# MIT-SPARK/Khronos

Measured on AMD Instinct MI355X. Metric: active-window frames/sec (+ Mvoxel-updates/sec) at 1280x720 RGB-D+labels, 2 cm voxels, higher is better.
Workload: dtype f32

## Files before the change

khronos_amd/csrc/khr_kernels_aux.h:

```cpp
#pragma once
#include <cstring>

#include "khr_device.h"

namespace khr {

#include "mc_table.inc"
__device__ int8_t g_mc_tri[256][16];
__device__ uint8_t g_mc_ntri[256];

constexpr uint64_t kSeedBit = kSeedFlag;

__global__ __launch_bounds__(256) void k_motion_pixels(DevMap m, DevParams p, DevFrame f, float md_max_range,
                                                      float min_z_world, uint64_t* __restrict__ keys, int ignore_epoch,
                                                      uint32_t* __restrict__ begin_band_count) {
  if (begin_band_count && blockIdx.x == 0) beginIntegrate(m, p.nvox, begin_band_count);
  const int i = blockIdx.x * blockDim.x + threadIdx.x;
  const bool in = i < f.W * f.H;
  uint64_t key = ~0ull;
  if (in)
    key = motionPixelKey(m, p, f.range[i], f.depth[i], i % f.W, i / f.W, f.fx, f.fy, f.cx, f.cy, f.Rw, f.tw, md_max_range,
                         min_z_world, ignore_epoch);
  if (in) keys[i] = key;
  const bool seed = (key != ~0ull) && (key & kSeedBit);
// ... 1548 lines not shown
  const uint32_t i = blockIdx.x * blockDim.x + threadIdx.x;
  if (i <= m.ht_mask) m.ht_keys[i] = kEmptyKey;
  if (i < m.capacity) {
    m.blk_flags[i] = 0u;
    m.mesh_desc[i] = MeshDesc{0u, 0u};
    m.free_slots[i] = i;
  }
  if (i < C_COUNT) m.counters[i] = i == C_N_FREE ? m.capacity : 0u;
  if (i < S_COUNT) m.stats[i] = 0ull;
}

__global__ __launch_bounds__(256) void k_block_flag_op(DevMap m, uint32_t and_mask, uint32_t or_mask) {
  const uint32_t s = blockIdx.x * blockDim.x + threadIdx.x;
  if (s >= m.counters[C_MAX_SLOT]) return;
  const uint32_t fl = m.blk_flags[s];
  if (fl & BLK_LIVE) m.blk_flags[s] = (fl & and_mask) | or_mask;
}

struct PackOut {
  float* dist;
  float* weight;
  uint32_t* color;
  uint64_t* last_obs;
  uint8_t* vflags;
  uint32_t* sem_label;
  uint64_t* last_occ;
  float* lik;
  int K, KS;
  uint64_t track_stamp;
};
template <int VPS>
__global__ __launch_bounds__(256) void k_pack_blocks(DevMap m, const uint32_t* __restrict__ slots, int n, PackOut o) {
  constexpr int NV = VPS * VPS * VPS;
  for (int b = blockIdx.x; b < n; b += gridDim.x) {
    const size_t src = static_cast<size_t>(slots[b]) * NV, dst = static_cast<size_t>(b) * NV;
    auto copy16 = [&](const void* s, void* d, size_t bytes) {
      const uint4* s4 = reinterpret_cast<const uint4*>(s);
      uint4* d4 = reinterpret_cast<uint4*>(d);
      for (size_t i = threadIdx.x; i < bytes / 16; i += 256) d4[i] = s4[i];
    };
    if (o.dist) copy16(m.dist + src, o.dist + dst, NV * 4);
    if (o.weight) copy16(m.weight + src, o.weight + dst, NV * 4);
    if (o.color) copy16(m.color + src, o.color + dst, NV * 4);
    if (o.last_obs) {
      const size_t sl = src / NV;
      for (int i = threadIdx.x; i < NV; i += 256) o.last_obs[dst + i] = lastObserved(m, sl, static_cast<uint32_t>(i), NV);
    }
    if (o.vflags) {
      const uint4* s4 = reinterpret_cast<const uint4*>(m.vflags + src);
      uint4* d4 = reinterpret_cast<uint4*>(o.vflags + dst);
      const uint32_t pm = VOX_PUBLIC_MASK * 0x01010101u;
      for (size_t i = threadIdx.x; i < NV / 16; i += 256) {
        const uint4 v = s4[i];
        d4[i] = make_uint4(v.x & pm, v.y & pm, v.z & pm, v.w & pm);
      }
    }
    if (o.sem_label) copy16(m.sem_label + src, o.sem_label + dst, NV * 4);
  }
}

__global__ __launch_bounds__(256) void k_snapshot_select(DevMap m, uint32_t* __restrict__ count, uint32_t* __restrict__ slots,
                                                        int4* __restrict__ index, uint32_t cap) {
  const uint32_t s = blockIdx.x * blockDim.x + threadIdx.x;
  bool take = false;
  if (s < m.counters[C_MAX_SLOT]) {
    const uint32_t fl = m.blk_flags[s];
    take = (fl & BLK_LIVE) && (fl & BLK_UPDATED);
  }
  const uint32_t pos = waveAggInc(count, take);
  if (take && pos < cap) {
    slots[pos] = s;
    index[pos] = m.blk_index[s];
  }
}
__global__ __launch_bounds__(256) void k_snapshot_index3(const int4* __restrict__ index, int32_t* __restrict__ out3, uint32_t n) {
  const uint32_t i = blockIdx.x * blockDim.x + threadIdx.x;
  if (i < n) {
    const int4 v = index[i];
    out3[3 * i] = v.x;
    out3[3 * i + 1] = v.y;
    out3[3 * i + 2] = v.z;
  }
}
template <int VPS>
__global__ __launch_bounds__(256) void k_snapshot_pack(DevMap m, const uint32_t* __restrict__ count, const uint32_t* __restrict__ slots,
                                                      uint32_t cap, PackOut o, volatile uint32_t* host_count, uint32_t ticket) {
  constexpr int NV = VPS * VPS * VPS;
  const uint32_t total = *count;
  const uint32_t n = min(total, cap);
  if (blockIdx.x == 0 && threadIdx.x == 0) {
    host_count[0] = total;
    __threadfence_system();
    host_count[1] = ticket;
    __threadfence_system();
  }
  for (uint32_t b = blockIdx.x; b < n; b += gridDim.x) {
    const size_t src = static_cast<size_t>(slots[b]) * NV, dst = static_cast<size_t>(b) * NV;
    auto copy16 = [&](const void* s, void* d, size_t bytes) {
      const uint4* s4 = reinterpret_cast<const uint4*>(s);
      uint4* d4 = reinterpret_cast<uint4*>(d);
      for (size_t i = threadIdx.x; i < bytes / 16; i += 256) d4[i] = s4[i];
    };
    if (o.dist) copy16(m.dist + src, o.dist + dst, NV * 4);
    if (o.weight) copy16(m.weight + src, o.weight + dst, NV * 4);
    if (o.color) copy16(m.color + src, o.color + dst, NV * 4);
    if (o.last_obs) {
      const size_t sl = src / NV;
      for (int i = threadIdx.x; i < NV; i += 256) o.last_obs[dst + i] = lastObserved(m, sl, static_cast<uint32_t>(i), NV);
    }
    if (o.vflags) {
      const uint4* s4 = reinterpret_cast<const uint4*>(m.vflags + src);
      uint4* d4 = reinterpret_cast<uint4*>(o.vflags + dst);
      const uint32_t pm = VOX_PUBLIC_MASK * 0x01010101u;
      for (size_t i = threadIdx.x; i < NV / 16; i += 256) {
        const uint4 v = s4[i];
        d4[i] = make_uint4(v.x & pm, v.y & pm, v.z & pm, v.w & pm);
      }
    }
    if (o.sem_label) copy16(m.sem_label + src, o.sem_label + dst, NV * 4);
    if (o.last_occ) {
      for (int i = threadIdx.x; i < NV; i += 256)
        o.last_occ[dst + i] = (m.vflags[src + i] & VOX_OCC) ? o.track_stamp : m.last_occ[src + i];
    }
    if (o.lik) {
      if (o.KS == o.K) copy16(m.lik + src * o.K, o.lik + dst * o.K, static_cast<size_t>(NV) * o.K * 4);
      else
        for (uint32_t i = threadIdx.x; i < static_cast<uint32_t>(NV) * static_cast<uint32_t>(o.K); i += 256) {
          const uint32_t v = i / static_cast<uint32_t>(o.K), k = i - v * static_cast<uint32_t>(o.K);
          o.lik[dst * o.K + i] = m.lik[(src + v) * o.KS + k];
        }
    }
  }
}

template <int VPS>
__global__ __launch_bounds__(256) void k_object_prune(DevMap m, DevParams p, float min_conf, float min_obs) {
  constexpr int NV = VPS * VPS * VPS;
  const uint32_t n_slots = m.counters[C_MAX_SLOT];
  uint32_t pruned = 0;
  for (uint32_t s = blockIdx.x; s < n_slots; s += gridDim.x) {
    if (!(m.blk_flags[s] & BLK_LIVE)) continue;
    const size_t o = static_cast<size_t>(s) * NV;
    bool touched = false;
    for (int lin = threadIdx.x; lin < NV; lin += 256) {
      const float d = m.dist[o + lin];
      if (d > 0.f) continue;
      float conf = 0.f;
      if (m.vflags[o + lin] & VOX_SEM_VALID) {
        const float l0 = m.lik[(static_cast<size_t>(s) * NV + lin) * p.KS + 0];
        const float l1 = m.lik[(static_cast<size_t>(s) * NV + lin) * p.KS + 1];
        const float total = l0 + l1;
        conf = total < min_obs ? -1.f : l1 / total;
      }
      if (conf < min_conf) {
        m.dist[o + lin] = p.trunc;
        ++pruned;
        touched = true;
      }
    }
    if (__any(touched) && (threadIdx.x & 63) == 0) atomicOr(&m.blk_flags[s], BLK_TRACK_DIRTY);
  }
#pragma unroll
  for (int o = 32; o > 0; o >>= 1) pruned += __shfl_down(pruned, o);
  if ((threadIdx.x & 63) == 0 && pruned) atomicAdd(&m.stats[S_PRUNED], static_cast<unsigned long long>(pruned));
}

constexpr int kDigestWords = 12;
__host__ __device__ inline uint64_t digestMix(uint64_t x) {
  x += 0x9e3779b97f4a7c15ull;
  x = (x ^ (x >> 30)) * 0xbf58476d1ce4e5b9ull;
  x = (x ^ (x >> 27)) * 0x94d049bb133111ebull;
  return x ^ (x >> 31);
}
__host__ __device__ inline uint64_t digestTerm(uint64_t key, uint32_t layer, uint64_t i, uint64_t value) {
  return digestMix(digestMix(key * 0x9e3779b97f4a7c15ull + static_cast<uint64_t>(layer) * 0x632be59bd9b4e019ull + i) ^ value);
}
__global__ __launch_bounds__(256) void k_map_digest(DevMap m, DevParams p, uint64_t track_stamp, unsigned long long* __restrict__ out) {
  const uint32_t n_slots = m.counters[C_MAX_SLOT];
  unsigned long long acc[kDigestWords];
#pragma unroll
  for (int l = 0; l < kDigestWords; ++l) acc[l] = 0ull;
  for (uint32_t s = blockIdx.x; s < n_slots; s += gridDim.x) {
    const uint32_t bf = m.blk_flags[s];
    if (!(bf & BLK_LIVE)) continue;
    const int4 bi = m.blk_index[s];
    const uint64_t key = packKey(bi.x, bi.y, bi.z);
    const size_t o = static_cast<size_t>(s) * p.nvox;
    for (int i = threadIdx.x; i < p.nvox; i += 256) {
      const uint8_t raw = m.vflags[o + i];
      acc[0] += digestTerm(key, 0, i, __float_as_uint(m.dist[o + i]));
      acc[1] += digestTerm(key, 1, i, __float_as_uint(m.weight[o + i]));
      acc[2] += digestTerm(key, 2, i, m.color[o + i]);
      const uint64_t lobs = p.with_tracking ? lastObserved(m, s, static_cast<uint32_t>(i), p.nvox) : 0ull;
      const uint64_t locc = p.with_tracking ? ((raw & VOX_OCC) ? track_stamp : m.last_occ[o + i]) : 0ull;
      acc[3] += digestTerm(key, 3, i, lobs);
      acc[4] += digestTerm(key, 4, i, locc);
      acc[5] += digestTerm(key, 5, i, raw & VOX_PUBLIC_MASK);
      acc[6] += digestTerm(key, 6, i, p.with_semantics ? m.sem_label[o + i] : 0u);
      if (p.with_semantics) {
        const bool valid = raw & VOX_SEM_VALID;
        const float* row = m.lik + (o + i) * p.KS;
        for (int k = 0; k < p.K; ++k)
          acc[7] += digestTerm(key, 7, static_cast<uint64_t>(k) * p.nvox + i, valid ? __float_as_uint(row[k]) : 0u);
      }
    }
    if (threadIdx.x == 0) {
      acc[8] += digestTerm(key, 8, 0, bf & 0xfu);
      acc[9] += digestMix(key);
      acc[10] += 1ull;
    }
  }
#pragma unroll
  for (int l = 0; l < kDigestWords; ++l) {
// ... 8 lines not shown
```

khronos_amd/csrc/khronos_amd.hip:

```cpp
#include <hip/hip_runtime.h>
#include <hip/hip_ext.h>
#include <hipcub/hipcub.hpp>

#include <algorithm>
#include <array>
#include <atomic>
#include <chrono>
#include <memory>
#include <mutex>
#include <cmath>
#include <cstdarg>
#include <cstdio>
#include <climits>
#include <cstring>
#include <cstdlib>
#include <functional>
#include <map>
#include <string>
#include <thread>
#include <tuple>
#include <unordered_map>
#include <vector>

#include "../../include/khronos_amd.h"
// ... 76 lines not shown
struct TimingRec {
  int which;
  Event a, b;
};

constexpr int kNumTimers = 13;
constexpr uint32_t kObjHead = 512;
constexpr uint32_t kCvHead = 8192;
constexpr int kGvReleaseGrid = 64;
constexpr uint32_t kCompCap = 1024, kCompHead = 64;

}

struct khr_ctx {
  khr_config cfg{};
  DevParams p{};
  DevMap m{};
  int device = 0;
  Stream stream;
  Stream aux_stream;
  Stream copy_stream;
  Stream snap_stream;
  Stream mc_stream;
  Stream h2d_stream;
  Event ev_aux, ev_aux_done;
  uint64_t aux_seq_issued = 0, aux_seq_done = 0, obj_seq = 0, cv_seq[3] = {0, 0, 0};
  std::vector<DevBuf<uint8_t>> allocs;
  std::vector<FrameSlot> slots;
  int next_slot = 0;
  std::unique_ptr<std::atomic<int>[]> slot_leases;
  uint32_t* d_work = nullptr;
  uint32_t* d_new = nullptr;
  uint32_t* d_ef = nullptr;
  uint32_t* d_trk_proc = nullptr;
  uint32_t* d_tick_work = nullptr;
  uint32_t* d_tick_counts = nullptr;
  uint32_t* d_tick_seeds = nullptr;
  PinnedBuf<uint32_t> h_tick;
  uint32_t tick_ticket = 0;
  std::vector<uint32_t> tick_seed_host;
  int tick_seed_n = 0, tick_seed_collected = 0;
  int tick_epoch = 0, motion_ignore_epoch = 0;
  unsigned long long* d_dbg = nullptr;
  unsigned long long* d_digest = nullptr;
  uint32_t* d_wg_stats = nullptr;
  bool defer_fold = false, fold_pending = false;
  int stream_priority = 0;
  unsigned char* d_fuse_sink = nullptr;
  DevBuf<uint32_t> d_pix_scratch;
  DevBuf<uint8_t> d_inst;
  uint4* d_work4 = nullptr;
  uint4* d_tick_work4 = nullptr;
  FuseFrame* d_tick_frames = nullptr;
  uint32_t* d_tick_mask = nullptr;
  bool tick_mask_dirty = false;
  uint32_t item_cap = 0;
  struct SnapArena {
    DevBuf<uint8_t> buf;
    PinnedBuf<uint32_t> count;
    volatile uint32_t* h_count() const { return count.get(); }
    int alloc(size_t bytes) {
      if (buf.alloc(bytes)) return fail(KHR_ENOMEM, "snapshot arena of %zu bytes", bytes);
      if (count.alloc(16)) {
        buf.reset();
        return fail(KHR_ENOMEM, "snapshot pinned words");
      }
      count[0] = count[1] = 0;
      return KHR_OK;
    }
  };
  struct SnapPool {
    std::mutex mu;
    std::vector<SnapArena> free;
    bool dead = false;
  };
  std::shared_ptr<SnapPool> snap_pool = std::make_shared<SnapPool>();
  struct FramePool {
    std::mutex mu;
    std::vector<DevBuf<uint8_t>> free;
    bool dead = false;
  };
  std::shared_ptr<FramePool> frame_pool = std::make_shared<FramePool>();
  khr_snapshot* pending_snapshot = nullptr;
  hipStream_t snap_stream_override = nullptr;
  Event ev_snap_fork, ev_snap_join;
  Event ev_mc_fork, ev_mc_join;
  bool fork_after_select = false;
  uint64_t explicit_blocks = 0;
  DevBuf<uint4> d_multi_list;
  DevBuf<uint32_t> d_frame_bits;
  PinnedBuf<FuseFrame> h_frames;
  DevBuf<FuseFrame> d_frames;
  Event ev_frames;
  uint32_t snap_ticket = 0;
  uint32_t wpb = 0;
  int fuse_zsplit = 2;
  DevBuf<uint64_t> d_halo_recs;
  const uint64_t* halo_view = nullptr;
  DevBuf<uint64_t> d_halo_keys;
  DevBuf<uint32_t> d_halo_vals;
  uint32_t halo_cap_total = 0, halo_mask = 0, halo_n = 0;
  DevBuf<uint32_t> d_mh_recs;
  const uint32_t* mh_view = nullptr;
  DevBuf<uint64_t> d_mh_keys;
  DevBuf<uint32_t> d_mh_vals;
  uint32_t mh_cap_total = 0, mh_mask = 0, mh_n = 0;
  uint8_t* d_mh_flag = nullptr;
  DevBuf<uint32_t> d_mh2_scratch;
  DevBuf<uint64_t> d_mh2_keys;
  DevBuf<uint32_t> d_mh2_offs;
  uint32_t mh2_ht = 0;
  bool mh_compact = false;
  PinnedBuf<uint32_t> h_pinned;
  uint32_t seed_ticket = 0;
  bool seed_publish_pending = false;
  bool seed_by_ticket = false;
  bool begin_in_ingest = false, begun = false;
  uint32_t fetch_ticket = 0;
  bool fetch_pending = false;
  uint32_t* d_fetch_done = nullptr;
  std::vector<uint32_t> fm_order;
  size_t fm_total = 0;
  uint64_t map_gen = 1, counters_gen = 0;
  int last_frame_slot = -1;
  PinnedBuf<void> h_stage;
  PinnedBuf<uint32_t> h_totals;
  PinnedBuf<void> h_up;
  Event ev_ingest;
  Event ev_up;
  hipStream_t ingest_stream = nullptr;
  struct AheadEntry { int slot; int ev; bool host; };
  std::vector<AheadEntry> ahead_q;
  Event ev_ahead[2];
  Event ev_ahead_h2d[2];
  int ahead_ev_next = 0;
  Event* h2d_ev_target = nullptr;
  Event ev_h2d;
  bool h2d_pending = false;
  bool host_input_pinned = false;
  uint64_t h2d_bytes = 0;
  int ef_parity = 0, ef_cur = 0;
  Event ev_seed;
  uint32_t last_removed = 0;
  khr_ctx* dep_src = nullptr;
  Event ev_dep, ev_dep_aux;
  uint64_t last_track_stamp = 0;
  bool removed_pending = false;
  int4* d_removed = nullptr;
  PinnedBuf<int4> h_removed_early;
  uint32_t* d_removed_early_n = nullptr;
  uint32_t removed_early_ticket = 0;
  bool removed_early = false;
  int* d_idx_staging = nullptr;
  uint64_t* d_keys = nullptr;
  uint32_t* d_pix = nullptr;
  void* d_cub_temp = nullptr;
  uint64_t* d_md_keys = nullptr;
  uint32_t *d_md_counts = nullptr, *d_md_ids = nullptr, *d_md_adj = nullptr;
  uint32_t* d_md_n = nullptr;
  uint64_t *d_md_seed_keys = nullptr, *d_md_bnd_keys = nullptr;
  uint32_t *d_md_seed_counts = nullptr, *d_md_bnd_counts = nullptr;
  int32_t *d_md_seed_final = nullptr, *d_md_bnd_final = nullptr;
  int32_t* d_md_bnd_deg = nullptr;
  unsigned long long* d_md_bnd_mask = nullptr;
  uint64_t n_seed_waits = 0, n_seed_waits_late = 0, seed_wait_max_us = 0, seed_wait_hist[8] = {0, 0, 0, 0, 0, 0, 0, 0};
  uint64_t seed_wait_late_us = 0, seed_wait_late_frame = 0, seed_wait_late_state = 0;
  bool last_ingest_on_aux = false;
// ... 3429 lines not shown
int khr_last_removed(khr_ctx* c, int32_t* removed, int64_t cap, int64_t* n_removed) {
  if (!c) return fail(KHR_EINVAL, "null ctx");
  return fetchRemoved(c, removed, cap, n_removed);
}

constexpr size_t kMaxAhead = 2;
static void cancelAhead(khr_ctx* c) {
  for (const auto& e : c->ahead_q) {
    c->slot_leases[e.slot].fetch_sub(1, std::memory_order_acq_rel);
    c->slots[e.slot].valid = false;
    if (c->obj_pending_slot == e.slot) c->obj_pending_slot = -1;
    if (e.host && c->ev_ahead_h2d[e.ev]) hipEventSynchronize(c->ev_ahead_h2d[e.ev]);
  }
  c->ahead_q.clear();
}

static bool pointerIs(const void* p, int where) {
  if (!p) return true;
  hipPointerAttribute_t at{};
  if (hipPointerGetAttributes(&at, p) != hipSuccess) {
    (void)hipGetLastError();
    return false;
  }
  if (where == 1) return at.type == hipMemoryTypeDevice || at.type == hipMemoryTypeManaged || at.type == hipMemoryTypeUnified;
  return at.type == hipMemoryTypeHost;
}

static int ingestAhead(khr_ctx* c, const khr_sensor* sensor, const khr_frame* frame, int on_device) {
  if (!c || !sensor || !frame) return fail(KHR_EINVAL, "null argument");
  if (c->ahead_q.size() >= kMaxAhead)
    return fail(KHR_ESTATE, "%zu frames handed over by khr_ingest_ahead are still waiting for khr_process_frame (khr_ingest_cancel drops them)", c->ahead_q.size());
  const int next = peekSlot(c);
  if (!c->cfg.with_tracking || c->slots.size() < 3 + c->ahead_q.size() || next < 0 || next == c->last_frame_slot) return KHR_ENOTFOUND;
  HIP_TRY(hipSetDevice(c->device));
  if (!pointerIs(frame->depth, on_device) || !pointerIs(frame->color, on_device) || !pointerIs(frame->label, on_device))
    return fail(KHR_EINVAL, on_device ? "khr_ingest_ahead: the frame's buffers must be device memory" : "khr_ingest_ahead_host: the frame's buffers must be page-locked host memory (hipHostMalloc / hipHostRegister)");
  const int evi = c->ahead_ev_next;
  for (const auto& e : c->ahead_q)
    if (e.ev == evi) return fail(KHR_ESTATE, "look-ahead event ring out of step");
  c->begin_in_ingest = false;
  hipStream_t conv_stream = c->aux_stream;
  if (!on_device) {
    if (!c->h2d_stream) KHR_TRY(createStream(c, c->h2d_stream));
    conv_stream = c->h2d_stream;
  }
  c->ingest_stream = conv_stream;
  c->host_input_pinned = !on_device;
  c->h2d_ev_target = &c->ev_ahead_h2d[evi];
  const int slot = khr_upload_frame(c, sensor, frame, on_device);
  c->h2d_ev_target = nullptr;
  c->host_input_pinned = false;
  c->ingest_stream = nullptr;
  if (slot < 0) return slot;
  auto undo = [&](int rc) {
    c->slots[slot].valid = false;
    if (!on_device && c->ev_ahead_h2d[evi]) hipEventSynchronize(c->ev_ahead_h2d[evi]);
    return rc;
  };
  if (c->ev_ahead[evi].ensure()) return undo(fail(KHR_EDEVICE, "hipEventCreate failed"));
  if (hipEventRecord(c->ev_ahead[evi], conv_stream) != hipSuccess) return undo(fail(KHR_EDEVICE, "hipEventRecord failed"));
  if (on_device) c->slots[slot].aux_seq = ++c->aux_seq_issued;
  if (on_device && c->obj_configured && c->obj_pending_slot < 0 && c->ahead_q.empty()) {
    const int rco = objectsLaunch(c, slot);
    if (rco) {
      if (c->obj_pending_slot == slot) c->obj_pending_slot = -1;
      return undo(rco);
    }
  }
  c->slot_leases[slot].fetch_add(1, std::memory_order_acq_rel);
  c->ahead_q.push_back({slot, evi, !on_device});
  c->ahead_ev_next ^= 1;
  return slot;
}

int khr_ingest_ahead(khr_ctx* c, const khr_sensor* sensor, const khr_frame* frame) { return ingestAhead(c, sensor, frame, 1); }
int khr_ingest_ahead_host(khr_ctx* c, const khr_sensor* sensor, const khr_frame* frame) { return ingestAhead(c, sensor, frame, 0); }
int khr_ingest_cancel(khr_ctx* c) {
  if (!c) return fail(KHR_EINVAL, "null ctx");
  if (c->ahead_q.empty()) return KHR_ENOTFOUND;
  cancelAhead(c);
  return KHR_OK;
}

int khr_process_frame(khr_ctx* c, const khr_sensor* sensor, const khr_frame* frame, int on_device, uint32_t flags,
                      int* n_clusters) {
  if (!c) return fail(KHR_EINVAL, "null ctx");
  HT("pf_enter");
  if (n_clusters) *n_clusters = 0;
  const bool motion = (flags & KHR_PF_MOTION) != 0;
  const bool objects = (flags & KHR_PF_OBJECTS) != 0;
  const bool ahead = (flags & KHR_PF_INGESTED) != 0;
  if (ahead && (c->ahead_q.empty() || !frame || !motion || !(flags & KHR_PF_INPUT_READY) ||
                c->slots[c->ahead_q.front().slot].meta.timestamp_ns != frame->timestamp_ns)) {
    cancelAhead(c);
    return fail(KHR_ESTATE, "KHR_PF_INGESTED: the oldest frame handed over by khr_ingest_ahead does not carry this stamp (or flags are missing); the handed-over frames were dropped");
  }
  if (!ahead && !c->ahead_q.empty()) return fail(KHR_ESTATE, "the frames handed over by khr_ingest_ahead have to be processed first (khr_ingest_cancel drops them)");
  const bool pinned_in = !on_device && (flags & KHR_PF_INPUT_PINNED) != 0;
  if (pinned_in && !ahead && frame && (!pointerIs(frame->depth, 0) || !pointerIs(frame->color, 0) || !pointerIs(frame->label, 0)))
    return fail(KHR_EINVAL, "KHR_PF_INPUT_PINNED: the frame's buffers must be page-locked host memory (hipHostMalloc / hipHostRegister)");
  struct Leave {
    khr_ctx* c;
    bool ok = false;
    ~Leave() {
      c->defer_fold = false;
      if (!ok && c->fold_pending) {
        hipLaunchKernelGGL(k_fuse_fold, dim3((c->m.capacity + 255) / 256), dim3(256), 0, c->stream, c->m.blk_flags, c->m.blk_band,
                           &c->m.counters[C_MAX_SLOT], static_cast<const uint32_t*>(nullptr));
        c->fold_pending = false;
      }
      if (c->h2d_pending) {
        hipEventSynchronize(c->ev_h2d);
        c->h2d_pending = false;
      }
      if (own_h2d) hipEventSynchronize(own_h2d);
    }
    hipEvent_t own_h2d = nullptr;
  } leave{c};
  const bool early = ahead || ((flags & KHR_PF_INPUT_READY) && (on_device || pinned_in) && motion && c->cfg.with_tracking &&
                               c->slots.size() >= (pinned_in ? 3u : 2u) && peekSlot(c) != c->last_frame_slot);
  int slot;
  int ahead_ev = 0;
  if (ahead) {
    const khr_ctx::AheadEntry e = c->ahead_q.front();
    c->ahead_q.erase(c->ahead_q.begin());
    slot = e.slot;
    ahead_ev = e.ev;
    if (e.host) leave.own_h2d = c->ev_ahead_h2d[e.ev];
    c->slot_leases[slot].fetch_sub(1, std::memory_order_acq_rel);
  } else {
    c->begin_in_ingest = !early;
    c->last_ingest_on_aux = early;
    c->ingest_stream = early ? c->aux_stream : nullptr;
    c->host_input_pinned = pinned_in;
    slot = khr_upload_frame(c, sensor, frame, on_device);
    c->host_input_pinned = false;
    c->ingest_stream = nullptr;
    c->begin_in_ingest = false;
    if (slot < 0) return slot;
  }
  c->last_frame_slot = slot;
  FrameSlot& s = c->slots[slot];
  const DevFrame f = makeDevFrame(c, s);
  int rc = KHR_OK;
  if (ahead) {
    c->begun = false;
    HIP_TRY(hipStreamWaitEvent(c->stream, c->ev_ahead[ahead_ev], 0));
  } else if (early) {
    c->begun = false;
    s.aux_seq = ++c->aux_seq_issued;
    HIP_TRY(hipEventRecord(c->ev_aux_done, c->aux_stream));
    HIP_TRY(hipStreamWaitEvent(c->stream, c->ev_aux_done, 0));
  }
  if (objects && !c->obj_configured) return fail(KHR_ESTATE, "KHR_PF_OBJECTS needs khr_configure_object_detector");
  if (objects && !early) {
    KHR_TRY(c->ev_ingest.ensure());
    HIP_TRY(hipEventRecord(c->ev_ingest, c->stream));
  }
  if (motion && (rc = motionLaunch(c, s, true, early))) return rc;
  if ((rc = integrateAlloc(c, s, f, 1))) return rc;
  HT("pf_alloc_launched");
  if (objects) {
    if (!(ahead && c->obj_pending_slot == slot)) {
      if (!early) HIP_TRY(hipStreamWaitEvent(c->aux_stream, c->ev_ingest, 0));
      if (ahead) HIP_TRY(hipStreamWaitEvent(c->aux_stream, c->ev_ahead[ahead_ev], 0));
      if ((rc = objectsLaunch(c, slot))) return rc;
    }
    HT("pf_objects_launched");
  }
  bool speculated = false;
  size_t spec_timer = static_cast<size_t>(-1), spec_end = 0;
  c->defer_fold = (flags & KHR_PF_TRACKING) && c->cfg.with_tracking;
  if (motion && c->cfg.with_tracking && !(c->md_seed_run && std::getenv("KHR_MD_NO_PRELAUNCH") == nullptr)) {
    const size_t n_pending = c->pending.size();
    rc = integrateUpdate(c, s, f, 1, 0, -1, nullptr, &c->m.counters[C_N_SEEDS]);
    if (rc) return rc;
    if (c->pending.size() > n_pending) spec_timer = n_pending;
    spec_end = c->pending.size();
    speculated = true;
  }
  bool have_seeds = false;
  if (motion) {
    c->md_defer_summary = true;
    c->md_summary_pending = -1;
    const int nc = motionFinish(c, s);
    c->md_defer_summary = false;
    if (nc < 0) return nc;
    if (n_clusters) *n_clusters = nc;
    have_seeds = c->cfg.with_tracking && c->h_pinned[0] != 0;
  }
  HT("pf_motion_done");
  if (speculated && have_seeds && spec_timer != static_cast<size_t>(-1))
    for (size_t i = spec_timer; i < spec_end && i < c->pending.size(); ++i) c->pending[i].which = -1;
  if (!speculated || have_seeds) {
    rc = integrateUpdate(c, s, f, 1, motion ? 1 : 0, -1);
    if (rc) return rc;
  }
  if (c->md_summary_pending >= 0) {
    const int pend = c->md_summary_pending;
    c->md_summary_pending = -1;
    if ((rc = clusterSummaryLaunch(c, s, pend))) return rc;
  }
  c->defer_fold = false;
  const bool mc_fork = (flags & KHR_PF_OUTPUT) && (flags & KHR_PF_TRACKING) && c->cfg.with_tracking;
  if (mc_fork) {
    if (!c->mc_stream) KHR_TRY(createStream(c, c->mc_stream));
    KHR_TRY(c->ev_mc_fork.ensure());
    KHR_TRY(c->ev_mc_join.ensure());
    c->fork_after_select = true;
  }
  rc = (flags & KHR_PF_TRACKING) ? khr_update_tracking(c, frame->timestamp_ns) : KHR_OK;
  c->fork_after_select = false;
  if (rc) return rc;
  const bool early_list = (flags & KHR_PF_OUTPUT) && c->cfg.with_tracking;
  if (mc_fork) {
    HIP_TRY(hipStreamWaitEvent(c->mc_stream, c->ev_mc_fork, 0));
    std::swap(c->stream, c->mc_stream);
    rc = khr_generate_mesh(c, 1, 1);
    std::swap(c->stream, c->mc_stream);
    if (rc) return rc;
    HIP_TRY(hipEventRecord(c->ev_mc_join, c->mc_stream));
  }
  HT("pf_update_launched");
  if (flags & KHR_PF_OUTPUT) {
    const bool snap = (flags & KHR_PF_SNAPSHOT) != 0;
    if (snap) {
      if (c->pending_snapshot) khr_snapshot_release(c->pending_snapshot);
      c->pending_snapshot = nullptr;
      if (!c->snap_stream) KHR_TRY(createStream(c, c->snap_stream));
      KHR_TRY(c->ev_snap_fork.ensure());
      KHR_TRY(c->ev_snap_join.ensure());
      HIP_TRY(hipEventRecord(c->ev_snap_fork, c->stream));
      HIP_TRY(hipStreamWaitEvent(c->snap_stream, c->ev_snap_fork, 0));
      const int64_t snap_cap = c->cfg.max_snapshot_blocks ? c->cfg.max_snapshot_blocks : 8192;
      c->snap_stream_override = c->snap_stream;
      rc = khr_snapshot_updated(c, KHR_SNAP_ALL, snap_cap, &c->pending_snapshot);
      c->snap_stream_override = nullptr;
      if (rc) return rc;
      HIP_TRY(hipEventRecord(c->ev_snap_join, c->snap_stream));
    }
    if (early_list && (rc = removedPublishLaunch(c))) return rc;
    if (mc_fork) HIP_TRY(hipStreamWaitEvent(c->stream, c->ev_mc_join, 0));
    else if ((rc = khr_generate_mesh(c, 1, 1))) return rc;
    if (snap) HIP_TRY(hipStreamWaitEvent(c->stream, c->ev_snap_join, 0));
    if (c->cfg.with_tracking) {
      if ((rc = resetInactiveLaunch(c, early_list, BLK_UPDATED))) return rc;
    } else if ((rc = khr_clear_updated(c))) {
      return rc;
    }
    c->removed_early = early_list;
    HT("pf_output_launched");
  }
  if (objects) {
    const int ns = objectsFinish(c, slot);
    if (ns < 0) return ns;
  }
  HT("pf_exit");
  leave.ok = true;
  return slot;
}

int khr_mark_all_inactive(khr_ctx* c) {
  if (!c) return fail(KHR_EINVAL, "null ctx");
  hipLaunchKernelGGL(k_block_flag_op, dim3(gridFor(c->m.capacity)), dim3(256), 0, c->stream, c->m, ~BLK_HAS_ACTIVE, BLK_TRACK_DIRTY);
  HIP_TRY(hipGetLastError());
  c->host_index_valid = false, ++c->map_gen;
  return KHR_OK;
}

int khr_clear_updated(khr_ctx* c) {
  if (!c) return fail(KHR_EINVAL, "null ctx");
  hipLaunchKernelGGL(k_block_flag_op, dim3(gridFor(c->m.capacity)), dim3(256), 0, c->stream, c->m, ~BLK_UPDATED, 0u);
  HIP_TRY(hipGetLastError());
  c->host_index_valid = false, ++c->map_gen;
  return KHR_OK;
}

int khr_allocate_blocks(khr_ctx* c, const int32_t* indices, int64_t n) {
  if (!c || (!indices && n > 0)) return fail(KHR_EINVAL, "null argument");
  if (n <= 0) return KHR_OK;
  HIP_TRY(hipSetDevice(c->device));
  std::vector<std::array<int32_t, 3>> v(n);
  for (int64_t i = 0; i < n; ++i) v[i] = {indices[3 * i], indices[3 * i + 1], indices[3 * i + 2]};
  std::sort(v.begin(), v.end());
  v.erase(std::unique(v.begin(), v.end()), v.end());
  const size_t bytes = sizeof(int32_t) * 3 * v.size();
  HT("ab_enter");
  if (c->ev_up) HIP_TRY(hipEventSynchronize(c->ev_up));
  KHR_TRY(c->ev_up.ensure());
  HT("ab_prev_upload_consumed");
  if (bytes > c->h_up.count()) {
    HIP_TRY(hipStreamSynchronize(c->stream));
    const size_t want = std::max<size_t>(2 * bytes, 1u << 16);
    if (c->h_up.reserve(want)) return fail(KHR_ENOMEM, "block index staging of %zu bytes", want);
  }
  std::memcpy(c->h_up, v.data(), bytes);
  HIP_TRY(hipMemsetAsync(&c->m.counters[C_N_NEW], 0, sizeof(uint32_t), c->stream));
  c->explicit_blocks += v.size();
  hipLaunchKernelGGL(k_alloc_list, dim3(gridFor(v.size())), dim3(256), 0, c->stream, c->m, static_cast<const int*>(c->h_up.dev()),
                     static_cast<int>(v.size()), c->d_new);
  HIP_TRY(hipEventRecord(c->ev_up, c->stream));
  hipLaunchKernelGGL(k_init_blocks, dim3(2048), dim3(256), 0, c->stream, c->m, c->p, c->d_new);
  HIP_TRY(hipGetLastError());
  c->host_index_valid = false, ++c->map_gen;
  return KHR_OK;
}

int khr_object_prune(khr_ctx* c, float min_confidence, float min_observations, int64_t* n_pruned) {
  if (!c) return fail(KHR_EINVAL, "null ctx");
  if (!c->cfg.with_semantics || c->p.K < 2) return fail(KHR_ESTATE, "object pruning needs a binary semantic layer");
  HIP_TRY(hipMemsetAsync(&c->m.stats[S_PRUNED], 0, sizeof(unsigned long long), c->stream));
  int rc = dispatchVps(c, [&](auto vps) {
    hipLaunchKernelGGL((k_object_prune<decltype(vps)::value>), dim3(kStreamGrid), dim3(256), 0, c->stream, c->m, c->p,
                       min_confidence, min_observations);
    return KHR_OK;
  });
  if (rc) return rc;
  if (n_pruned) {
    unsigned long long np = 0;
    HIP_TRY(hipMemcpyAsync(&np, &c->m.stats[S_PRUNED], sizeof(np), hipMemcpyDeviceToHost, c->stream));
    HIP_TRY(hipStreamSynchronize(c->stream));
    *n_pruned = static_cast<int64_t>(np);
// ... 1222 lines not shown
  auto carve = [&](size_t b) { uint8_t* p = cur; cur += (b + 15) / 16 * 16; return p; };
  PackOut o{};
  if (last_observed && trk) o.last_obs = reinterpret_cast<uint64_t*>(carve(tot * 8));
  if (distance) o.dist = reinterpret_cast<float*>(carve(tot * 4));
  if (weight) o.weight = reinterpret_cast<float*>(carve(tot * 4));
  if (color_rgba) o.color = reinterpret_cast<uint32_t*>(carve(tot * 4));
  if (sem_label && sem) o.sem_label = reinterpret_cast<uint32_t*>(carve(tot * 4));
  if (voxel_flags) o.vflags = carve(tot);
  uint32_t* d_slots = reinterpret_cast<uint32_t*>(carve(sizeof(uint32_t) * n));
  hipError_t e = hipMemcpyAsync(d_slots, slots.data(), sizeof(uint32_t) * n, hipMemcpyHostToDevice, c->stream);
  if (e == hipSuccess) {
    rc = dispatchVps(c, [&](auto vps) {
      hipLaunchKernelGGL((k_pack_blocks<decltype(vps)::value>), dim3(static_cast<unsigned>(std::min<int64_t>(n, 4096))), dim3(256), 0,
                         c->stream, c->m, d_slots, static_cast<int>(n), o);
      return KHR_OK;
    });
    auto D = [&](void* dst, const void* src, size_t b) { if (e == hipSuccess && dst && src) e = hipMemcpyAsync(dst, src, b, hipMemcpyDeviceToHost, c->stream); };
    D(distance, o.dist, tot * 4);
    D(weight, o.weight, tot * 4);
    D(color_rgba, o.color, tot * 4);
    D(last_observed, o.last_obs, tot * 8);
    D(voxel_flags, o.vflags, tot);
    D(sem_label, o.sem_label, tot * 4);
    if (e == hipSuccess) e = hipStreamSynchronize(c->stream);
  }
  if (e != hipSuccess) return fail(KHR_EDEVICE, "download_updated failed: %s", hipGetErrorString(e));
  if (rc) return rc;
  if (last_observed && !trk) std::memset(last_observed, 0, tot * 8);
  if (sem_label && !sem) std::memset(sem_label, 0, tot * 4);
  return n;
}

struct khr_snapshot {
  khr_ctx* ctx = nullptr;
  std::shared_ptr<khr_ctx::SnapPool> pool;
  int device = 0;
  khr_ctx::SnapArena arena;
  uint32_t fields = 0, cap = 0, nvox = 0, ticket = 0;
  uint32_t* d_count = nullptr;
  uint32_t* d_slots = nullptr;
  int4* d_index = nullptr;
  PackOut o{};
  int64_t n = -1;
  int64_t total = -1;
  Event ev_packed;
  Event ev_copied;
  bool copying = false;
  int32_t* d_index3 = nullptr;
};

static size_t snapBytes(uint32_t fields, size_t cap, size_t nvox, bool trk, bool sem, size_t K) {
  auto al = [](size_t b) { return (b + 255) / 256 * 256; };
  size_t b = 256 + al(cap * 4) + al(cap * 16) + al(cap * 12);
  if (fields & KHR_SNAP_DISTANCE) b += al(cap * nvox * 4);
  if (fields & KHR_SNAP_WEIGHT) b += al(cap * nvox * 4);
  if (fields & KHR_SNAP_COLOR) b += al(cap * nvox * 4);
  if ((fields & KHR_SNAP_LAST_OBSERVED) && trk) b += al(cap * nvox * 8);
  if (fields & KHR_SNAP_FLAGS) b += al(cap * nvox);
  if ((fields & KHR_SNAP_LABEL) && sem) b += al(cap * nvox * 4);
  if ((fields & KHR_SNAP_LAST_OCCUPIED) && trk) b += al(cap * nvox * 8);
  if ((fields & KHR_SNAP_LIKELIHOODS) && sem) b += al(cap * nvox * 4 * K);
  return b;
}

int khr_reserve_snapshots(khr_ctx* c, uint32_t fields, int64_t cap_blocks, int n_arenas) {
  if (!c || !(fields & KHR_SNAP_EVERYTHING) || n_arenas < 0 || n_arenas > 16) return fail(KHR_EINVAL, "bad argument");
  HIP_TRY(hipSetDevice(c->device));
  const size_t cap = cap_blocks > 0 ? static_cast<size_t>(std::min<int64_t>(cap_blocks, c->m.capacity)) : c->m.capacity;
  const size_t need = snapBytes(fields, cap, c->p.nvox, c->cfg.with_tracking, c->cfg.with_semantics, static_cast<size_t>(c->p.K));
  size_t have = 0;
  {
    std::lock_guard<std::mutex> lock(c->snap_pool->mu);
    for (const auto& a : c->snap_pool->free) have += a.buf.count() >= need ? 1 : 0;
  }
  for (size_t i = have; i < static_cast<size_t>(n_arenas); ++i) {
    khr_ctx::SnapArena a;
    KHR_TRY(a.alloc(need));
    std::lock_guard<std::mutex> lock(c->snap_pool->mu);
    c->snap_pool->free.push_back(std::move(a));
  }
  return KHR_OK;
}

int khr_snapshot_updated(khr_ctx* c, uint32_t fields, int64_t cap_blocks, khr_snapshot** out) {
  if (!c || !out || !(fields & KHR_SNAP_EVERYTHING)) return fail(KHR_EINVAL, "bad argument");
  *out = nullptr;
  HIP_TRY(hipSetDevice(c->device));
  const bool trk = c->cfg.with_tracking, sem = c->cfg.with_semantics;
  const size_t cap = cap_blocks > 0 ? static_cast<size_t>(std::min<int64_t>(cap_blocks, c->m.capacity)) : c->m.capacity;
  const size_t nvox = c->p.nvox;
  const size_t need = snapBytes(fields, cap, nvox, trk, sem, static_cast<size_t>(c->p.K));
  auto snap = std::make_unique<khr_snapshot>();
  {
    auto& fr = c->snap_pool->free;
    std::lock_guard<std::mutex> lock(c->snap_pool->mu);
    size_t best = fr.size();
    for (size_t i = 0; i < fr.size(); ++i)
      if (fr[i].buf.count() >= need && (best == fr.size() || fr[i].buf.count() < fr[best].buf.count())) best = i;
    if (best < fr.size()) {
      snap->arena = std::move(fr[best]);
      fr.erase(fr.begin() + static_cast<long>(best));
    }
  }
  if (!snap->arena.buf) KHR_TRY(snap->arena.alloc(need));
  snap->ctx = c;
  snap->pool = c->snap_pool;
  snap->device = c->device;
  snap->fields = fields;
  snap->cap = static_cast<uint32_t>(cap);
  snap->nvox = static_cast<uint32_t>(nvox);
  snap->ticket = ++c->snap_ticket;
  if (snap->ticket == 0) snap->ticket = ++c->snap_ticket;
  uint8_t* cur = snap->arena.buf;
  auto carve = [&](size_t b) { uint8_t* p = cur; cur += (b + 255) / 256 * 256; return p; };
  snap->d_count = reinterpret_cast<uint32_t*>(carve(256));
  snap->d_slots = reinterpret_cast<uint32_t*>(carve(cap * 4));
  snap->d_index = reinterpret_cast<int4*>(carve(cap * 16));
  snap->d_index3 = reinterpret_cast<int32_t*>(carve(cap * 12));
  if (fields & KHR_SNAP_DISTANCE) snap->o.dist = reinterpret_cast<float*>(carve(cap * nvox * 4));
  if (fields & KHR_SNAP_WEIGHT) snap->o.weight = reinterpret_cast<float*>(carve(cap * nvox * 4));
  if (fields & KHR_SNAP_COLOR) snap->o.color = reinterpret_cast<uint32_t*>(carve(cap * nvox * 4));
  if ((fields & KHR_SNAP_LAST_OBSERVED) && trk) snap->o.last_obs = reinterpret_cast<uint64_t*>(carve(cap * nvox * 8));
  if (fields & KHR_SNAP_FLAGS) snap->o.vflags = carve(cap * nvox);
  if ((fields & KHR_SNAP_LABEL) && sem) snap->o.sem_label = reinterpret_cast<uint32_t*>(carve(cap * nvox * 4));
  if ((fields & KHR_SNAP_LAST_OCCUPIED) && trk) snap->o.last_occ = reinterpret_cast<uint64_t*>(carve(cap * nvox * 8));
  if ((fields & KHR_SNAP_LIKELIHOODS) && sem) snap->o.lik = reinterpret_cast<float*>(carve(cap * nvox * 4 * static_cast<size_t>(c->p.K)));
  snap->o.K = c->p.K;
  snap->o.KS = c->p.KS;
  snap->o.track_stamp = c->last_track_stamp;
  hipStream_t st = c->snap_stream_override ? c->snap_stream_override : c->stream;
  hipError_t e = hipMemsetAsync(snap->d_count, 0, 4, st);
  int rc_ev = KHR_OK;
  if (e == hipSuccess) {
    hipLaunchKernelGGL(k_snapshot_select, dim3(gridFor(c->m.capacity)), dim3(256), 0, st, c->m, snap->d_count, snap->d_slots,
                       snap->d_index, snap->cap);
    dispatchVps(c, [&](auto vps) {
      KHR_LAUNCH_TIMED_ON(12, st, (k_snapshot_pack<decltype(vps)::value>), dim3(2048), dim3(256), c->m, snap->d_count, snap->d_slots,
                          snap->cap, snap->o, snap->arena.count.dev(), snap->ticket);
      return KHR_OK;
    });
    e = hipGetLastError();
    if (e == hipSuccess) rc_ev = snap->ev_packed.ensure();
    if (e == hipSuccess && rc_ev == KHR_OK) e = hipEventRecord(snap->ev_packed, st);
  }
  if (e != hipSuccess || rc_ev != KHR_OK) {
    std::lock_guard<std::mutex> lock(c->snap_pool->mu);
    c->snap_pool->free.push_back(std::move(snap->arena));
    return rc_ev != KHR_OK ? rc_ev : fail(KHR_EDEVICE, "snapshot launch failed: %s", hipGetErrorString(e));
  }
  *out = snap.release();
  return KHR_OK;
}

int khr_take_snapshot(khr_ctx* c, khr_snapshot** out) {
  if (!c || !out) return fail(KHR_EINVAL, "null argument");
  *out = c->pending_snapshot;
  c->pending_snapshot = nullptr;
  return *out ? KHR_OK : KHR_ENOTFOUND;
}

static int snapshotWait(khr_snapshot* s) {
  if (s->n >= 0) return KHR_OK;
  const auto t0 = std::chrono::steady_clock::now();
  while (s->arena.h_count()[1] != s->ticket) {
    if (std::chrono::steady_clock::now() - t0 > std::chrono::seconds(20)) return fail(KHR_EDEVICE, "snapshot was never produced (stream stuck?)");
    std::this_thread::yield();
  }
  s->total = s->arena.h_count()[0];
  s->n = std::min<int64_t>(s->total, s->cap);
  return KHR_OK;
}

int khr_snapshot_poll(khr_snapshot* s) {
  if (!s) return fail(KHR_EINVAL, "null snapshot");
  return (s->n >= 0 || s->arena.h_count()[1] == s->ticket) ? 1 : 0;
}

int64_t khr_snapshot_num_blocks(khr_snapshot* s) {
  if (!s) return fail(KHR_EINVAL, "null snapshot");
  const int rc = snapshotWait(s);
  return rc ? rc : s->total;
}

static int64_t snapshotDownload(khr_snapshot* s, int32_t* indices, float* distance, float* weight, uint8_t* color_rgba,
                                uint64_t* last_observed, uint8_t* voxel_flags, uint32_t* sem_label, uint64_t* last_occupied,
                                float* likelihoods, int64_t cap_blocks) {
  if (!s) return fail(KHR_EINVAL, "null snapshot");
  int rc = snapshotWait(s);
  if (rc) return rc;
  if (s->total > s->cap) return fail(KHR_ENOMEM, "%lld updated blocks, snapshot capacity %u", static_cast<long long>(s->total), s->cap);
  const int64_t n = s->n;
  if (n > cap_blocks) return fail(KHR_EINVAL, "%lld blocks in the snapshot, cap %lld", static_cast<long long>(n), static_cast<long long>(cap_blocks));
  if (n == 0) return 0;
  {
    std::lock_guard<std::mutex> lock(s->pool->mu);
    if (s->pool->dead) return fail(KHR_ESTATE, "the snapshot's context has been destroyed");
  }
  khr_ctx* c = s->ctx;
  HIP_TRY(hipSetDevice(c->device));
  if (s->copying) return fail(KHR_ESTATE, "an asynchronous download of this snapshot is in flight (khr_snapshot_download_end first)");
  HIP_TRY(hipEventSynchronize(s->ev_packed));
  const size_t nv = s->nvox;
  if (indices) {
    std::vector<int4> idx(static_cast<size_t>(n));
    HIP_TRY(hipMemcpy(idx.data(), s->d_index, sizeof(int4) * n, hipMemcpyDeviceToHost));
    for (int64_t i = 0; i < n; ++i) {
      indices[3 * i] = idx[i].x;
      indices[3 * i + 1] = idx[i].y;
      indices[3 * i + 2] = idx[i].z;
    }
  }
  hipError_t e = hipSuccess;
  auto field = [&](void* dst, const void* src, size_t elem) {
    if (e == hipSuccess && dst && src) e = hipMemcpyAsync(dst, src, static_cast<size_t>(n) * nv * elem, hipMemcpyDeviceToHost, c->stream);
  };
  field(distance, s->o.dist, 4);
  field(weight, s->o.weight, 4);
  field(color_rgba, s->o.color, 4);
  field(last_observed, s->o.last_obs, 8);
  field(voxel_flags, s->o.vflags, 1);
  field(sem_label, s->o.sem_label, 4);
  field(last_occupied, s->o.last_occ, 8);
  field(likelihoods, s->o.lik, 4 * static_cast<size_t>(s->o.K));
  if (e == hipSuccess) e = hipStreamSynchronize(c->stream);
  if (e != hipSuccess) return fail(KHR_EDEVICE, "snapshot download failed: %s", hipGetErrorString(e));
  return n;
}

int64_t khr_snapshot_download(khr_snapshot* s, int32_t* indices, float* distance, float* weight, uint8_t* color_rgba,
                              uint64_t* last_observed, uint8_t* voxel_flags, uint32_t* sem_label, int64_t cap_blocks) {
  return snapshotDownload(s, indices, distance, weight, color_rgba, last_observed, voxel_flags, sem_label, nullptr, nullptr, cap_blocks);
}

// ... 312 lines not shown
```

Before: 4127.

## Split snapshot pack into early/late layers and parallelize pack over layers

```diff
diff --git a/khronos_amd/csrc/khr_kernels_aux.h b/khronos_amd/csrc/khr_kernels_aux.h
--- a/khronos_amd/csrc/khr_kernels_aux.h
+++ b/khronos_amd/csrc/khr_kernels_aux.h
@@ -1654,53 +1654,102 @@
     out3[3 * i + 2] = v.z;
   }
 }
+template <int R>
+__device__ inline void packCopy16(const uint4* __restrict__ s, uint4* __restrict__ d, uint32_t n16, uint32_t mask) {
+  for (uint32_t i = threadIdx.x; i < n16; i += 256u * R) {
+    uint4 v[R];
+#pragma unroll
+    for (int k = 0; k < R; ++k) {
+      v[k] = make_uint4(0u, 0u, 0u, 0u);
+      if (i + 256u * k < n16) v[k] = s[i + 256u * k];
+    }
+#pragma unroll
+    for (int k = 0; k < R; ++k)
+      if (i + 256u * k < n16) d[i + 256u * k] = make_uint4(v[k].x & mask, v[k].y & mask, v[k].z & mask, v[k].w & mask);
+  }
+}
+template <int R>
+__device__ inline void packLastObserved(const ulonglong2* __restrict__ obs, const uint64_t* __restrict__ lobs,
+                                        ulonglong2* __restrict__ d, uint32_t nvox) {
+  const uint32_t np = nvox >> 1;
+  for (uint32_t p = threadIdx.x; p < np; p += 256u * R) {
+    ulonglong2 w[R], v[R];
+#pragma unroll
+    for (int k = 0; k < R; ++k) {
+      w[k] = make_ulonglong2(0ull, 0ull);
+      if (p + 256u * k < np) w[k] = obs[(p + 256u * k) >> 5];
+    }
+#pragma unroll
+    for (int k = 0; k < R; ++k) {
+      const uint32_t lin = 2u * (p + 256u * k);
+      const uint32_t lazy = (p + 256u * k < np) ? static_cast<uint32_t>(w[k].x >> (lin & 63u)) & 3u : 3u;
+      v[k] = make_ulonglong2(w[k].y, w[k].y);
+      if (lazy == 0u) {
+        v[k] = *reinterpret_cast<const ulonglong2*>(lobs + lin);
+      } else {
+        if (!(lazy & 1u)) v[k].x = lobs[lin];
+        if (!(lazy & 2u)) v[k].y = lobs[lin + 1];
+      }
+    }
+#pragma unroll
+    for (int k = 0; k < R; ++k)
+      if (p + 256u * k < np) d[p + 256u * k] = v[k];
+  }
+}
 template <int VPS>
 __global__ __launch_bounds__(256) void k_snapshot_pack(DevMap m, const uint32_t* __restrict__ count, const uint32_t* __restrict__ slots,
                                                       uint32_t cap, PackOut o, volatile uint32_t* host_count, uint32_t ticket) {
-  constexpr int NV = VPS * VPS * VPS;
+  constexpr uint32_t NV = VPS * VPS * VPS;
+  static_assert(NV % 64 == 0, "a block's layers are whole 16-byte rows and whole lazy-stamp groups");
   const uint32_t total = *count;
   const uint32_t n = min(total, cap);
-  if (blockIdx.x == 0 && threadIdx.x == 0) {
+  if (host_count && blockIdx.x == 0 && threadIdx.x == 0) {
     host_count[0] = total;
     __threadfence_system();
     host_count[1] = ticket;
     __threadfence_system();
   }
-  for (uint32_t b = blockIdx.x; b < n; b += gridDim.x) {
-    const size_t src = static_cast<size_t>(slots[b]) * NV, dst = static_cast<size_t>(b) * NV;
-    auto copy16 = [&](const void* s, void* d, size_t bytes) {
-      const uint4* s4 = reinterpret_cast<const uint4*>(s);
-      uint4* d4 = reinterpret_cast<uint4*>(d);
-      for (size_t i = threadIdx.x; i < bytes / 16; i += 256) d4[i] = s4[i];
+  enum : uint32_t { L_OBS, L_LIK, L_OCC, L_DIST, L_WEIGHT, L_COLOR, L_LABEL, L_FLAGS };
+  uint32_t code = 0, n_layers = 0;
+  auto add = [&](const void* ptr, uint32_t layer) {
+    if (ptr) code |= layer << (4u * n_layers++);
+  };
+  add(o.last_obs, L_OBS), add(o.lik, L_LIK), add(o.last_occ, L_OCC), add(o.dist, L_DIST), add(o.weight, L_WEIGHT);
+  add(o.color, L_COLOR), add(o.sem_label, L_LABEL), add(o.vflags, L_FLAGS);
+  if (n == 0) return;
+  const uint64_t n_items = static_cast<uint64_t>(n) * n_layers;
+  for (uint64_t it = blockIdx.x; it < n_items; it += gridDim.x) {
+    const uint32_t li = static_cast<uint32_t>(it / n), b = static_cast<uint32_t>(it - static_cast<uint64_t>(li) * n);
+    const uint32_t layer = (code >> (4u * li)) & 15u;
+    const size_t slot = slots[b];
+    const size_t src = slot * NV, dst = static_cast<size_t>(b) * NV;
+    auto copy = [&](const void* s, void* d, uint32_t bytes, uint32_t mask) {
+      packCopy16<4>(reinterpret_cast<const uint4*>(s), reinterpret_cast<uint4*>(d), bytes / 16u, mask);
     };
-    if (o.dist) copy16(m.dist + src, o.dist + dst, NV * 4);
-    if (o.weight) copy16(m.weight + src, o.weight + dst, NV * 4);
-    if (o.color) copy16(m.color + src, o.color + dst, NV * 4);
-    if (o.last_obs) {
-      const size_t sl = src / NV;
-      for (int i = threadIdx.x; i < NV; i += 256) o.last_obs[dst + i] = lastObserved(m, sl, static_cast<uint32_t>(i), NV);
-    }
-    if (o.vflags) {
-      const uint4* s4 = reinterpret_cast<const uint4*>(m.vflags + src);
-      uint4* d4 = reinterpret_cast<uint4*>(o.vflags + dst);
-      const uint32_t pm = VOX_PUBLIC_MASK * 0x01010101u;
-      for (size_t i = threadIdx.x; i < NV / 16; i += 256) {
-        const uint4 v = s4[i];
-        d4[i] = make_uint4(v.x & pm, v.y & pm, v.z & pm, v.w & pm);
-      }
-    }
-    if (o.sem_label) copy16(m.sem_label + src, o.sem_label + dst, NV * 4);
-    if (o.last_occ) {
-      for (int i = threadIdx.x; i < NV; i += 256)
-        o.last_occ[dst + i] = (m.vflags[src + i] & VOX_OCC) ? o.track_stamp : m.last_occ[src + i];
-    }
-    if (o.lik) {
-      if (o.KS == o.K) copy16(m.lik + src * o.K, o.lik + dst * o.K, static_cast<size_t>(NV) * o.K * 4);
-      else
-        for (uint32_t i = threadIdx.x; i < static_cast<uint32_t>(NV) * static_cast<uint32_t>(o.K); i += 256) {
-          const uint32_t v = i / static_cast<uint32_t>(o.K), k = i - v * static_cast<uint32_t>(o.K);
-          o.lik[dst * o.K + i] = m.lik[(src + v) * o.KS + k];
+    switch (layer) {
+      case L_DIST: copy(m.dist + src, o.dist + dst, NV * 4u, ~0u); break;
+      case L_WEIGHT: copy(m.weight + src, o.weight + dst, NV * 4u, ~0u); break;
+      case L_COLOR: copy(m.color + src, o.color + dst, NV * 4u, ~0u); break;
+      case L_LABEL: copy(m.sem_label + src, o.sem_label + dst, NV * 4u, ~0u); break;
+      case L_FLAGS: copy(m.vflags + src, o.vflags + dst, NV, VOX_PUBLIC_MASK * 0x01010101u); break;
+      case L_OBS:
+        packLastObserved<4>(m.obs + slot * (NV >> 6), m.last_obs + src, reinterpret_cast<ulonglong2*>(o.last_obs + dst), NV);
+        break;
+      case L_OCC:
+        for (uint32_t i = threadIdx.x; i < NV; i += 256)
+          o.last_occ[dst + i] = (m.vflags[src + i] & VOX_OCC) ? o.track_stamp : m.last_occ[src + i];
+        break;
+      default:
+        if (o.KS == o.K) {
+          packCopy16<4>(reinterpret_cast<const uint4*>(m.lik + src * o.K), reinterpret_cast<uint4*>(o.lik + dst * o.K),
+                        NV / 4u * static_cast<uint32_t>(o.K), ~0u);
+        } else {
+          for (uint32_t i = threadIdx.x; i < NV * static_cast<uint32_t>(o.K); i += 256) {
+            const uint32_t v = i / static_cast<uint32_t>(o.K), k = i - v * static_cast<uint32_t>(o.K);
+            o.lik[dst * o.K + i] = m.lik[(src + v) * o.KS + k];
+          }
         }
+        break;
     }
   }
 }
diff --git a/khronos_amd/csrc/khronos_amd.hip b/khronos_amd/csrc/khronos_amd.hip
--- a/khronos_amd/csrc/khronos_amd.hip
+++ b/khronos_amd/csrc/khronos_amd.hip
@@ -182,7 +182,6 @@
   };
   std::shared_ptr<FramePool> frame_pool = std::make_shared<FramePool>();
   khr_snapshot* pending_snapshot = nullptr;
-  hipStream_t snap_stream_override = nullptr;
   Event ev_snap_fork, ev_snap_join;
   Event ev_mc_fork, ev_mc_join;
   bool fork_after_select = false;
@@ -3778,6 +3777,12 @@
   return KHR_OK;
 }
 
+static int snapshotCreate(khr_ctx* c, uint32_t fields, int64_t cap_blocks, khr_snapshot** out);
+static void snapshotAbandon(khr_ctx* c, khr_snapshot* snap, hipStream_t st);
+static int snapshotSelectLaunch(khr_ctx* c, khr_snapshot* snap, hipStream_t st);
+static int snapshotPackLaunch(khr_ctx* c, khr_snapshot* snap, hipStream_t st, uint32_t layers, bool publish);
+static int snapshotSeal(khr_snapshot* snap, hipStream_t st);
+
 int khr_process_frame(khr_ctx* c, const khr_sensor* sensor, const khr_frame* frame, int on_device, uint32_t flags,
                       int* n_clusters) {
   if (!c) return fail(KHR_EINVAL, "null ctx");
@@ -3810,8 +3815,10 @@
         c->h2d_pending = false;
       }
       if (own_h2d) hipEventSynchronize(own_h2d);
+      if (snap) snapshotAbandon(c, snap, c->snap_stream);
     }
     hipEvent_t own_h2d = nullptr;
+    khr_snapshot* snap = nullptr;
   } leave{c};
   const bool early = ahead || ((flags & KHR_PF_INPUT_READY) && (on_device || pinned_in) && motion && c->cfg.with_tracking &&
                                c->slots.size() >= (pinned_in ? 3u : 2u) && peekSlot(c) != c->last_frame_slot);
@@ -3926,14 +3933,26 @@
       if (!c->snap_stream) KHR_TRY(createStream(c, c->snap_stream));
       KHR_TRY(c->ev_snap_fork.ensure());
       KHR_TRY(c->ev_snap_join.ensure());
+      const int64_t snap_cap = c->cfg.max_snapshot_blocks ? c->cfg.max_snapshot_blocks : 8192;
+      const uint32_t late_layers = mc_fork ? (KHR_SNAP_FLAGS | KHR_SNAP_LAST_OCCUPIED) : 0u;
+      KHR_TRY(snapshotCreate(c, KHR_SNAP_ALL, snap_cap, &leave.snap));
+      if (mc_fork) {
+        HIP_TRY(hipStreamWaitEvent(c->snap_stream, c->ev_mc_fork, 0));
+        KHR_TRY(snapshotSelectLaunch(c, leave.snap, c->snap_stream));
+        KHR_TRY(snapshotPackLaunch(c, leave.snap, c->snap_stream, KHR_SNAP_EVERYTHING & ~late_layers, true));
+      }
       HIP_TRY(hipEventRecord(c->ev_snap_fork, c->stream));
       HIP_TRY(hipStreamWaitEvent(c->snap_stream, c->ev_snap_fork, 0));
-      const int64_t snap_cap = c->cfg.max_snapshot_blocks ? c->cfg.max_snapshot_blocks : 8192;
-      c->snap_stream_override = c->snap_stream;
-      rc = khr_snapshot_updated(c, KHR_SNAP_ALL, snap_cap, &c->pending_snapshot);
-      c->snap_stream_override = nullptr;
-      if (rc) return rc;
+      if (mc_fork) {
+        KHR_TRY(snapshotPackLaunch(c, leave.snap, c->snap_stream, late_layers, false));
+      } else {
+        KHR_TRY(snapshotSelectLaunch(c, leave.snap, c->snap_stream));
+        KHR_TRY(snapshotPackLaunch(c, leave.snap, c->snap_stream, KHR_SNAP_EVERYTHING, true));
+      }
       HIP_TRY(hipEventRecord(c->ev_snap_join, c->snap_stream));
+      KHR_TRY(snapshotSeal(leave.snap, c->snap_stream));
+      c->pending_snapshot = leave.snap;
+      leave.snap = nullptr;
     }
     if (early_list && (rc = removedPublishLaunch(c))) return rc;
     if (mc_fork) HIP_TRY(hipStreamWaitEvent(c->stream, c->ev_mc_join, 0));
@@ -5322,10 +5341,7 @@
   return KHR_OK;
 }
 
-int khr_snapshot_updated(khr_ctx* c, uint32_t fields, int64_t cap_blocks, khr_snapshot** out) {
-  if (!c || !out || !(fields & KHR_SNAP_EVERYTHING)) return fail(KHR_EINVAL, "bad argument");
-  *out = nullptr;
-  HIP_TRY(hipSetDevice(c->device));
+static int snapshotCreate(khr_ctx* c, uint32_t fields, int64_t cap_blocks, khr_snapshot** out) {
   const bool trk = c->cfg.with_tracking, sem = c->cfg.with_semantics;
   const size_t cap = cap_blocks > 0 ? static_cast<size_t>(std::min<int64_t>(cap_blocks, c->m.capacity)) : c->m.capacity;
   const size_t nvox = c->p.nvox;
@@ -5368,27 +5384,69 @@
   snap->o.K = c->p.K;
   snap->o.KS = c->p.KS;
   snap->o.track_stamp = c->last_track_stamp;
-  hipStream_t st = c->snap_stream_override ? c->snap_stream_override : c->stream;
-  hipError_t e = hipMemsetAsync(snap->d_count, 0, 4, st);
-  int rc_ev = KHR_OK;
-  if (e == hipSuccess) {
-    hipLaunchKernelGGL(k_snapshot_select, dim3(gridFor(c->m.capacity)), dim3(256), 0, st, c->m, snap->d_count, snap->d_slots,
-                       snap->d_index, snap->cap);
-    dispatchVps(c, [&](auto vps) {
-      KHR_LAUNCH_TIMED_ON(12, st, (k_snapshot_pack<decltype(vps)::value>), dim3(2048), dim3(256), c->m, snap->d_count, snap->d_slots,
-                          snap->cap, snap->o, snap->arena.count.dev(), snap->ticket);
-      return KHR_OK;
-    });
-    e = hipGetLastError();
-    if (e == hipSuccess) rc_ev = snap->ev_packed.ensure();
-    if (e == hipSuccess && rc_ev == KHR_OK) e = hipEventRecord(snap->ev_packed, st);
-  }
-  if (e != hipSuccess || rc_ev != KHR_OK) {
+  *out = snap.release();
+  return KHR_OK;
+}
+
+static void snapshotAbandon(khr_ctx* c, khr_snapshot* snap, hipStream_t st) {
+  if (!snap) return;
+  if (st) (void)hipStreamSynchronize(st);
+  {
     std::lock_guard<std::mutex> lock(c->snap_pool->mu);
     c->snap_pool->free.push_back(std::move(snap->arena));
-    return rc_ev != KHR_OK ? rc_ev : fail(KHR_EDEVICE, "snapshot launch failed: %s", hipGetErrorString(e));
-  }
-  *out = snap.release();
+  }
+  delete snap;
+}
+
+static int snapshotSelectLaunch(khr_ctx* c, khr_snapshot* snap, hipStream_t st) {
+  HIP_TRY(hipMemsetAsync(snap->d_count, 0, 4, st));
+  hipLaunchKernelGGL(k_snapshot_select, dim3(gridFor(c->m.capacity)), dim3(256), 0, st, c->m, snap->d_count, snap->d_slots,
+                     snap->d_index, snap->cap);
+  HIP_TRY(hipGetLastError());
+  return KHR_OK;
+}
+
+static int snapshotPackLaunch(khr_ctx* c, khr_snapshot* snap, hipStream_t st, uint32_t layers, bool publish) {
+  PackOut o = snap->o;
+  if (!(layers & KHR_SNAP_DISTANCE)) o.dist = nullptr;
+  if (!(layers & KHR_SNAP_WEIGHT)) o.weight = nullptr;
+  if (!(layers & KHR_SNAP_COLOR)) o.color = nullptr;
+  if (!(layers & KHR_SNAP_LAST_OBSERVED)) o.last_obs = nullptr;
+  if (!(layers & KHR_SNAP_FLAGS)) o.vflags = nullptr;
+  if (!(layers & KHR_SNAP_LABEL)) o.sem_label = nullptr;
+  if (!(layers & KHR_SNAP_LAST_OCCUPIED)) o.last_occ = nullptr;
+  if (!(layers & KHR_SNAP_LIKELIHOODS)) o.lik = nullptr;
+  uint32_t* const host_count = publish ? snap->arena.count.dev() : nullptr;
+  dispatchVps(c, [&](auto vps) {
+    KHR_LAUNCH_TIMED_ON(12, st, (k_snapshot_pack<decltype(vps)::value>), dim3(2048), dim3(256), c->m, snap->d_count, snap->d_slots,
+                        snap->cap, o, host_count, snap->ticket);
+    return KHR_OK;
+  });
+  HIP_TRY(hipGetLastError());
+  return KHR_OK;
+}
+
+static int snapshotSeal(khr_snapshot* snap, hipStream_t st) {
+  KHR_TRY(snap->ev_packed.ensure());
+  HIP_TRY(hipEventRecord(snap->ev_packed, st));
+  return KHR_OK;
+}
+
+int khr_snapshot_updated(khr_ctx* c, uint32_t fields, int64_t cap_blocks, khr_snapshot** out) {
+  if (!c || !out || !(fields & KHR_SNAP_EVERYTHING)) return fail(KHR_EINVAL, "bad argument");
+  *out = nullptr;
+  HIP_TRY(hipSetDevice(c->device));
+  khr_snapshot* snap = nullptr;
+  KHR_TRY(snapshotCreate(c, fields, cap_blocks, &snap));
+  hipStream_t st = c->stream;
+  int rc = snapshotSelectLaunch(c, snap, st);
+  if (rc == KHR_OK) rc = snapshotPackLaunch(c, snap, st, KHR_SNAP_EVERYTHING, true);
+  if (rc == KHR_OK) rc = snapshotSeal(snap, st);
+  if (rc != KHR_OK) {
+    snapshotAbandon(c, snap, st);
+    return rc;
+  }
+  *out = snap;
   return KHR_OK;
 }
 
```

Result: no change. 4125 (median of 2 runs) (-0.0%).
